# vinhisreal/YOLO-LitePi

Hardware: AMD Instinct MI355X
Metric: images/sec end-to-end (det+NMS+clf) 640x640 batch64 (higher is better)
Workload: dtype f16; 1 GPU; configs[2]: full det+NMS+ROI+ShuffleNetV2 pipeline, fp16, batch=64/GPU, 640x640, inputs resident in HBM; classifier=ShuffleNetV2 x1.0, 91 classes, seeded random weights, 64x64 ROIs, min_area=50, max_det=300, steps_in_flight=3, distinct_input_batches=4, global_batch=64, boxes_pre_area_filter_rank0=413

## Files before the change

yolo-litepi_amd/csrc/classifier.cpp:

```cpp
#include "classifier.h"

#include <algorithm>
#include <cmath>
#include <cstdlib>

namespace lp {

static const int kStageRepeats[3] = {4, 8, 4};
static const int kStageOut[3] = {116, 232, 464};

Classifier::Classifier(int prec, int impl, int max_rois, int num_classes, int input_size)
    : prec_(prec), impl_(impl), maxR_(max_rois), ncls_(num_classes), S_(input_size) {}

static View make_view(const DevBuf& buf, size_t es, int coff, int C, int pitch, int H, int W) {
  View v;
  v.base = static_cast<char*>(buf.p) + (size_t)coff * es;
  v.C = C; v.pitch = pitch; v.H = H; v.W = W;
  return v;
}

View Classifier::act_view(const Act& a, int coff, int C) const {
  return make_view(a.mem, prec_ == LP_FP16 ? 2 : 4, coff, C < 0 ? a.C : C, a.C, a.H, a.W);
}

// ... 143 lines not shown
        if (use_fused_) { upload_f32(fused_s2_[s].dw1, w); upload_f32(fused_s2_[s].dw1b, b); }
        Folded q = fold(sd, p + "branch1.2", p + "branch1.3");
        LP_CHECK(q.co == bf && q.ci == inp && q.k == 1, LP_ERR_ARG, "%sbranch1.2 shape", p.c_str());
        expand_pw(q, lin, 0, bfp, w, b, lin.Cp(), 0);
        B.b1_pw = add_pw(p + "branch1.2", w, b, lin.Cp(), bfp, ACT_RELU, Ho);
        if (use_fused_) { upload_u16(fused_s2_[s].pwb1, pack_fused_pw(w, bfp, lin.Cp())); upload_f32(fused_s2_[s].pwb1b, b); }
        Folded a1 = fold(sd, p + "branch2.0", p + "branch2.1");
        LP_CHECK(a1.co == bf && a1.ci == inp, LP_ERR_ARG, "%sbranch2.0 shape", p.c_str());
        expand_pw(a1, lin, 0, bfp, w, b, lin.Cp(), 0);
        B.b2_pw1 = add_pw(p + "branch2.0", w, b, lin.Cp(), bfp, ACT_RELU, Hin);
        if (use_fused_) { upload_u16(fused_s2_[s].pw1, pack_fused_pw(w, bfp, lin.Cp())); upload_f32(fused_s2_[s].pw1b, b); }
        b1dw_elems = std::max(b1dw_elems, (size_t)Ho * Ho * lin.Cp());
        b1_elems = std::max(b1_elems, (size_t)Ho * Ho * bfp);
        t1_elems = std::max(t1_elems, (size_t)Hin * Hin * bfp);
      } else {
        Folded a1 = fold(sd, p + "branch2.0", p + "branch2.1");
        LP_CHECK(a1.co == bf && a1.ci == bf, LP_ERR_ARG, "%sbranch2.0 shape", p.c_str());
        expand_pw(a1, lout, bf, bfp, w, b, bfp, bfp);
        B.b2_pw1 = add_pw(p + "branch2.0", w, b, bfp, bfp, ACT_RELU, Ho);
        t1_elems = std::max(t1_elems, (size_t)Ho * Ho * bfp);
        if (use_fused_) {
          fused_[s].emplace_back();
          upload_u16(fused_[s].back().w1, pack_fused_pw(w, bfp, bfp));
          upload_f32(fused_[s].back().b1, b);
        }
      }
      Layout lmid;
      lmid.C = bf;
      Folded d2 = fold(sd, p + "branch2.3", p + "branch2.4");
      LP_CHECK(d2.co == bf && d2.ci == 1 && d2.k == 3, LP_ERR_ARG, "%sbranch2.3 shape", p.c_str());
      expand_dw(d2, lmid, 0, bfp, 0, w, b);
      B.b2_dw = add_dw(p + "branch2.3", w, b, bfp, B.stride);
      if (use_fused_ && B.stride == 1) { upload_f32(fused_[s].back().dw, w); upload_f32(fused_[s].back().dwb, b); }
      if (use_fused_ && B.stride == 2) { upload_f32(fused_s2_[s].dw2, w); upload_f32(fused_s2_[s].dw2b, b); }
      Folded a2 = fold(sd, p + "branch2.5", p + "branch2.6");
      LP_CHECK(a2.co == bf && a2.ci == bf, LP_ERR_ARG, "%sbranch2.5 shape", p.c_str());
      expand_pw(a2, lmid, 0, bfp, w, b, bfp, 0);
      B.b2_pw2 = add_pw(p + "branch2.5", w, b, bfp, bfp, ACT_RELU, Ho);
      if (use_fused_ && B.stride == 1) { upload_u16(fused_[s].back().w2, pack_fused_pw(w, bfp, bfp)); upload_f32(fused_[s].back().b2, b); }
      if (use_fused_ && B.stride == 2) { upload_u16(fused_s2_[s].pw2, pack_fused_pw(w, bfp, bfp)); upload_f32(fused_s2_[s].pw2b, b); }
      t2_elems = std::max(t2_elems, (size_t)Ho * Ho * bfp);
      blocks_.push_back(B);
      inp = oup;
      lin = lout;
    }
    H = Ho;
    alloc_act(a_stage_[s][0], 2 * bfp, H, H);
    alloc_act(a_stage_[s][1], 2 * bfp, H, H);
  }
  if (use_fused_) {
    LP_CHECK(half_c_[0] == 58 && half_cp_[0] == 64 && half_c_[1] == 116 && half_cp_[1] == 128 && half_c_[2] == 232 && half_cp_[2] == 240,
             LP_ERR_STATE, "fused classifier kernels are built for ShuffleNetV2 x1.0 widths");
    a_x3_.alloc((size_t)maxR_ * 16 * 256 * 2);
  }
  const size_t es = prec_ == LP_FP16 ? 2 : 4;
  a_t1_.mem.alloc((size_t)maxR_ * t1_elems * es);
  a_t2_.mem.alloc((size_t)maxR_ * t2_elems * es);
  a_b1dw_.mem.alloc((size_t)maxR_ * b1dw_elems * es);
  a_b1_.mem.alloc((size_t)maxR_ * b1_elems * es);

  {
    Folded f = fold(sd, "conv5.0", "conv5.1");
    LP_CHECK(f.co == 1024 && f.ci == 464 && f.k == 1, LP_ERR_ARG, "conv5 must be 464->1024 1x1");
    std::vector<float> w, b;
    expand_pw(f, lin, 0, 1024, w, b, lin.Cp(), 0);
    conv5_ = add_pw("conv5.0", w, b, lin.Cp(), 1024, ACT_RELU, H);
    if (use_fused_) {
      LP_CHECK(H == 2, LP_ERR_STATE, "fused head expects a 2x2 stage-4 map");
      head_cin_p_ = lin.Cp();
      upload_u16(head_w5_, pack_fused_pw(w, 1024, lin.Cp()));
      upload_f32(head_b5_, b);
    }
    alloc_act(a_conv5_, 1024, H, H);
    alloc_act(a_mean_, 1024, 1, 1);
    const NamedTensor& fw = need(sd, "fc.weight");
    const NamedTensor& fb = need(sd, "fc.bias");
    LP_CHECK(fw.shape.size() == 2 && fw.shape[0] == ncls_ && fw.shape[1] == 1024 && (int)fb.numel() == ncls_, LP_ERR_ARG,
             "fc must be Linear(1024, %d), got [%lld,%lld]", ncls_, (long long)(fw.shape.size() ? fw.shape[0] : 0),
             (long long)(fw.shape.size() > 1 ? fw.shape[1] : 0));
    const int cp = round_up(ncls_, 8);
    lpitch_ = round_up(ncls_, 16);
    std::vector<float> w2((size_t)cp * 1024, 0.f), b2(cp, 0.f);
    for (int o = 0; o < ncls_; ++o) {
      memcpy(&w2[(size_t)o * 1024], fw.data + (size_t)o * 1024, 1024 * 4);
      b2[o] = fb.data[o];
    }
    fc_ = add_pw("fc", w2, b2, 1024, cp, ACT_NONE, 1);
    if (use_fused_) {
      head_nc_p_ = round_up(ncls_, 16);
      std::vector<float> wf((size_t)head_nc_p_ * 1024, 0.f), bf2(head_nc_p_, 0.f);
      for (int o = 0; o < ncls_; ++o) {
        memcpy(&wf[(size_t)o * 1024], fw.data + (size_t)o * 1024, 1024 * 4);
        bf2[o] = fb.data[o];
      }
      upload_u16(head_wfc_, pack_fused_pw(wf, head_nc_p_, 1024));
      upload_f32(head_bfc_, bf2);
    }
    d_logits_.alloc((size_t)maxR_ * lpitch_ * 4);
  }
  loaded_ = true;
}

void Classifier::forward(const uint8_t* rgb, const int* d_R, hipStream_t st, Profiler* prof, const Post* post) {
  LP_CHECK(loaded_, LP_ERR_STATE, "classifier not loaded");
  const size_t es = prec_ == LP_FP16 ? 2 : 4;
  const char* sfx = prec_ == LP_FP16 ? "_f16" : "_f32";
  const double esd = (double)es;
  auto P0 = [&]() { if (prof) prof->begin(st); };
  auto P1 = [&](const char* kname, const std::string& layer, double flops, double bytes) {
    if (prof) prof->end(st, std::string(kname) + sfx, layer, flops, bytes, true);
  };
  auto run_pw = [&](int idx, const View& in, const View& out, const View* x1, int half_c, int half_cp, int out_f32) {
    const ConvLayer& c = *pws_[idx];
    ConvIO io;
    io.in = in; io.out = out; io.N = maxR_; io.m_dyn = d_R; io.out_f32 = out_f32;
    if (x1) { io.x1 = *x1; io.half_c = half_c; io.half_cp = half_cp; }
    P0();
    c.launch(io, st);
    const double px = (double)out.H * out.W;
    P1(c.impl == IMPL_NAIVE ? "conv_naive" : "conv1x1_mfma", c.name, 2.0 * c.Cin * c.Cout * px,
       px * (c.Cin + c.Cout * (x1 ? 2.0 : 1.0)) * esd);
  };
  auto run_dw = [&](int idx, const View& in, const View& out) {
    const DwLayer& d = dws_[idx];
    P0();
    launch_dwconv3x3(prec_, in, out, d.w.as<float>(), d.b.as<float>(), d.stride, d_R, maxR_, st);
    P1("dwconv3x3", d.name, 2.0 * 9 * d.C * out.H * out.W, ((double)in.H * in.W + (double)out.H * out.W) * d.C * esd);
  };

  static const bool two_launch = getenv("LITEPI_CLS_LAYERWISE") == nullptr;
  if (use_fused_ && two_launch) {
    auto s2w = [](const FusedS2& f) {
      FusedS2W w;
      w.dw1 = f.dw1.as<float>(); w.dw1b = f.dw1b.as<float>(); w.pwb1 = f.pwb1.as<u32x4_t>(); w.pwb1b = f.pwb1b.as<float>();
      w.pw1 = f.pw1.as<u32x4_t>(); w.pw1b = f.pw1b.as<float>(); w.dw2 = f.dw2.as<float>(); w.dw2b = f.dw2b.as<float>();
      w.pw2 = f.pw2.as<u32x4_t>(); w.pw2b = f.pw2b.as<float>();
      return w;
    };
    auto s1w = [](const FusedW& f) {
      FusedBlockW w;
      w.w1 = f.w1.as<u32x4_t>(); w.b1 = f.b1.as<float>(); w.dw = f.dw.as<float>(); w.dwb = f.dwb.as<float>();
      w.w2 = f.w2.as<u32x4_t>(); w.b2 = f.b2.as<float>();
      return w;
    };
    ClsFrontArgs fa;
    memset(&fa, 0, sizeof(fa));
    fa.rgb = rgb; fa.m_dyn = d_R; fa.out = a_x3_.p;
    fa.stem_w = stem_frag_.as<u32x4_t>(); fa.stem_b = stem_bias4_.as<float>();
    fa.s20 = s2w(fused_s2_[0]);
    for (int q = 0; q < 3; ++q) fa.s2[q] = s1w(fused_[0][q]);
    fa.s30 = s2w(fused_s2_[1]);
    P0();
    launch_cls_front(fa, maxR_, st);
    P1("cls_front", "conv1..stage3.0", 2.0 * (0.66e6 + 2.10e6 + 0.60e6), 12288.0 + 8192.0);
    ClsBackArgs ba;
    memset(&ba, 0, sizeof(ba));
    ba.in = a_x3_.p; ba.m_dyn = d_R;
    for (int q = 0; q < 7; ++q) ba.s3[q] = s1w(fused_[1][q]);
    ba.s40 = s2w(fused_s2_[2]);
    for (int q = 0; q < 3; ++q) ba.s4[q] = s1w(fused_[2][q]);
    ba.w5 = head_w5_.as<u32x4_t>(); ba.b5 = head_b5_.as<float>();
    ba.wfc = head_wfc_.as<u32x4_t>(); ba.bfc = head_bfc_.as<float>();
    ba.nc = ncls_; ba.nc_p = head_nc_p_;
    ba.logits = d_logits_.as<float>(); ba.logits_pitch = lpitch_;
    if (post) {
      ba.probs = post->probs; ba.ids = post->ids; ba.dets = post->dets; ba.max_det = post->max_det;
      ba.roi_img = post->roi_img; ba.roi_slot = post->roi_slot;
    }
    P0();
    launch_cls_back(ba, maxR_, st);
    P1("cls_back", "stage3.1..softmax", 2.0 * (3.86e6 + 2.63e6 + 1.90e6 + 1024.0 * ncls_), 8192.0 + ncls_ * 4.0);
    return;
  }
  P0();
  launch_cls_stem(prec_, rgb, stem_w_.as<float>(), stem_b_.as<float>(), 24, act_view(a_stem_), S_, d_R, maxR_, st);
  P1("cls_stem", "conv1", 2.0 * 27 * 24 * a_stem_.H * a_stem_.W, (double)S_ * S_ * 3 + (double)a_stem_.H * a_stem_.W * 24 * esd);
  P0();
  launch_maxpool3x3s2(prec_, act_view(a_stem_), act_view(a_pool_), d_R, maxR_, st);
  P1("maxpool3x3s2", "maxpool", 0.0, ((double)a_stem_.H * a_stem_.W + (double)a_pool_.H * a_pool_.W) * 24 * esd);

  View x = act_view(a_pool_);
  size_t bi = 0;
  for (int s = 0; s < 3; ++s) {
    const int bf = half_c_[s], bfp = half_cp_[s];
    for (int r = 0; r < kStageRepeats[s]; ++r, ++bi) {
      const Block& B = blocks_[bi];
      if (use_fused_ && r == 1) {
        Act& dstf = a_stage_[s][1];
        FusedStageArgs fa;
        memset(&fa, 0, sizeof(fa));
        fa.in = x.base; fa.out = dstf.mem.p; fa.m_dyn = d_R;
        fa.nblk = kStageRepeats[s] - 1;
        for (int q = 0; q < fa.nblk; ++q) {
          const FusedW& fw = fused_[s][q];
          fa.blk[q].w1 = fw.w1.as<u32x4_t>(); fa.blk[q].b1 = fw.b1.as<float>();
          fa.blk[q].dw = fw.dw.as<float>(); fa.blk[q].dwb = fw.dwb.as<float>();
          fa.blk[q].w2 = fw.w2.as<u32x4_t>(); fa.blk[q].b2 = fw.b2.as<float>();
        }
        fa.HW = dstf.H * dstf.W; fa.W = dstf.W; fa.bf = bf; fa.bfp = bfp; fa.group = 64 / fa.HW;
        fa.in_pitch = x.pitch; fa.out_pitch = dstf.C;
        P0();
        launch_fused_stage(fa, maxR_, st);
        const double px = (double)fa.HW;
        P1("shuffle_stage_fused", fmt("stage%d.1-%d", s + 2, kStageRepeats[s] - 1),
           fa.nblk * (2.0 * 2.0 * bfp * bfp + 2.0 * 9 * bfp) * px, 2.0 * px * 2 * bfp * esd);
        x = act_view(dstf);
        bi += kStageRepeats[s] - 1;
        break;
      }
      Act& dst = a_stage_[s][r & 1];
      const int Ho = dst.H;
      const View out = act_view(dst);
      const View t2 = make_view(a_t2_.mem, es, 0, bfp, bfp, Ho, Ho);
      if (B.stride == 2) {
        const View b1dw = make_view(a_b1dw_.mem, es, 0, x.C, x.C, Ho, Ho);
        const View b1 = make_view(a_b1_.mem, es, 0, bfp, bfp, Ho, Ho);
        const View t1 = make_view(a_t1_.mem, es, 0, bfp, bfp, x.H, x.W);
        run_dw(B.b1_dw, x, b1dw);
        run_pw(B.b1_pw, b1dw, b1, nullptr, 0, 0, 0);
        run_pw(B.b2_pw1, x, t1, nullptr, 0, 0, 0);
        run_dw(B.b2_dw, t1, t2);
        run_pw(B.b2_pw2, t2, out, &b1, bf, bfp, 0);
      } else {
        const View x1 = View{x.base, bfp, x.pitch, x.H, x.W};
        const View x2 = View{static_cast<char*>(x.base) + (size_t)bfp * es, bfp, x.pitch, x.H, x.W};
        const View t1 = make_view(a_t1_.mem, es, 0, bfp, bfp, Ho, Ho);
        run_pw(B.b2_pw1, x2, t1, nullptr, 0, 0, 0);
        run_dw(B.b2_dw, t1, t2);
        run_pw(B.b2_pw2, t2, out, &x1, bf, bfp, 0);
      }
      x = out;
    }
  }
  if (use_fused_) {
    FusedHeadArgs ha;
    memset(&ha, 0, sizeof(ha));
    ha.in = x.base; ha.m_dyn = d_R; ha.in_pitch = x.pitch; ha.cin_p = head_cin_p_;
    ha.w5 = head_w5_.as<u32x4_t>(); ha.b5 = head_b5_.as<float>();
    ha.wfc = head_wfc_.as<u32x4_t>(); ha.bfc = head_bfc_.as<float>();
    ha.nc = ncls_; ha.nc_p = head_nc_p_;
    ha.logits = d_logits_.as<float>(); ha.logits_pitch = lpitch_;
    if (post) {
      ha.probs = post->probs; ha.ids = post->ids; ha.dets = post->dets; ha.max_det = post->max_det;
      ha.roi_img = post->roi_img; ha.roi_slot = post->roi_slot;
    }
    P0();
    launch_fused_head(ha, maxR_, st);
    P1("cls_head_fused", "conv5+mean+fc+softmax", 4.0 * 2.0 * head_cin_p_ * 1024 + 2.0 * 1024 * head_nc_p_,
       4.0 * head_cin_p_ * esd + ncls_ * 4.0);
    return;
  }
  run_pw(conv5_, x, act_view(a_conv5_), nullptr, 0, 0, 0);
  P0();
  launch_spatial_mean(prec_, act_view(a_conv5_), act_view(a_mean_), d_R, maxR_, st);
  P1("spatial_mean", "mean", 0.0, (double)(a_conv5_.H * a_conv5_.W + 1) * 1024 * esd);
  View lg;
  lg.base = d_logits_.p; lg.C = lpitch_; lg.pitch = lpitch_; lg.H = 1; lg.W = 1;
  run_pw(fc_, act_view(a_mean_), lg, nullptr, 0, 0, 1);
}

}
```

yolo-litepi_amd/csrc/cls_net.hip:

```cpp
#include "cls_net.h"

namespace lp {

typedef _Float16 half_t;
typedef _Float16 half8 __attribute__((ext_vector_type(8)));
typedef _Float16 half4 __attribute__((ext_vector_type(4)));
typedef _Float16 half2v __attribute__((ext_vector_type(2)));
typedef float floatx4 __attribute__((ext_vector_type(4)));
typedef uint32_t u32x4 __attribute__((ext_vector_type(4)));

#define CN_THREADS 512
#define CN_WAVES 8

#define BF2 58
#define BFP2 64
#define BF3 116
#define BFP3 128
#define BF4 232
#define BFP4 240

template <int SMAX>
__device__ __forceinline__ void wload(u32x4 (&af)[SMAX], const u32x4_t* __restrict__ w, int t, int S, int lane) {
#pragma unroll
  for (int s = 0; s < SMAX; ++s) {
// ... 42 lines not shown
}

template <int C, int WIN, int WOUT, int STRIDE>
__device__ __forceinline__ void dwconv(const char* in, int irow, char* out, int orow, const float* __restrict__ w,
                                       const float* __restrict__ b, int nroi, int tid) {
  constexpr int CG = C / 8;
  const int items = nroi * WOUT * WOUT * CG;
  for (int i = tid; i < items; i += CN_THREADS) {
    const int cg = i % CG, px = i / CG;
    const int r = px / (WOUT * WOUT), pp = px - r * (WOUT * WOUT);
    const int oy = pp / WOUT, ox = pp - oy * WOUT;
    float acc[8];
    {
      const floatx4 b0 = *reinterpret_cast<const floatx4*>(b + cg * 8), b1 = *reinterpret_cast<const floatx4*>(b + cg * 8 + 4);
#pragma unroll
      for (int j = 0; j < 4; ++j) { acc[j] = b0[j]; acc[4 + j] = b1[j]; }
    }
#pragma unroll 1
    for (int ky = 0; ky < 3; ++ky) {
      const int iy = oy * STRIDE - 1 + ky;
      if (iy < 0 || iy >= WIN) continue;
      const char* rowp = in + ((r * WIN + iy) * WIN) * irow + cg * 16;
      const float* wrow = w + (ky * 3) * C + cg * 8;
#pragma unroll
      for (int kx = 0; kx < 3; ++kx) {
        const int ix = ox * STRIDE - 1 + kx;
        const bool ok = ix >= 0 && ix < WIN;
        u32x4 raw = u32x4{0u, 0u, 0u, 0u};
        if (ok) raw = *reinterpret_cast<const u32x4*>(rowp + ix * irow);
        const half8 v = __builtin_bit_cast(half8, raw);
        const floatx4 w0 = *reinterpret_cast<const floatx4*>(wrow + kx * C);
        const floatx4 w1 = *reinterpret_cast<const floatx4*>(wrow + kx * C + 4);
#pragma unroll
        for (int j = 0; j < 4; ++j) {
          acc[j] = fmaf((float)v[j], w0[j], acc[j]);
          acc[4 + j] = fmaf((float)v[4 + j], w1[j], acc[4 + j]);
        }
      }
    }
    half8 o;
#pragma unroll
    for (int j = 0; j < 8; ++j) o[j] = (half_t)acc[j];
    *reinterpret_cast<half8*>(out + px * orow + cg * 16) = o;
  }
}

__device__ __forceinline__ int shuffle_phys(int l, int bf, int bfp) { return l < bf ? l : bfp + (l - bf); }

template <int BFP, int NB>
__device__ __forceinline__ void stage_biases(float* BI, const FusedBlockW* blk, int tid) {
  constexpr int Q = BFP / 4;
  for (int i = tid; i < NB * 2 * Q; i += CN_THREADS) {
    const int b = i / (2 * Q), rem = i - b * 2 * Q, which = rem / Q, j = rem - which * Q;
    const float* src = which ? blk[b].b2 : blk[b].b1;
    *reinterpret_cast<floatx4*>(BI + (size_t)(b * 2 + which) * BFP + 4 * j) = *reinterpret_cast<const floatx4*>(src + 4 * j);
  }
}

template <int C>
__device__ __forceinline__ void stage_dw(float* dst, const float* __restrict__ w, const float* __restrict__ b, int tid) {
  constexpr int Q = 10 * C / 4;
  for (int i = tid; i < Q; i += CN_THREADS)
    *reinterpret_cast<floatx4*>(dst + 4 * i) = i < 9 * C / 4 ? *reinterpret_cast<const floatx4*>(w + 4 * i) : *reinterpret_cast<const floatx4*>(b + 4 * (i - 9 * C / 4));
}

template <int BF, int BFP, int W, int PT, int ROUNDS, bool PREF = true>
__device__ __forceinline__ void s1_block(char* X, int xrow, char* T1, char* T2, int trow, const FusedBlockW& bw, const u32x4_t* w1n, int nroi,
                                         int p0, int tile0, int tstride, u32x4 (&f1)[ROUNDS][BFP / 32 + ((BFP % 32) ? 1 : 0)], int tid, float* DW, const float* BI) {
  constexpr int TT = BFP / 16, S = BFP / 32 + ((BFP % 32) ? 1 : 0);
  const int lane = tid & 63;
  const int g = lane >> 4, col = lane & 15;
  constexpr int NDW4 = 10 * BFP / 4, DWPT = (NDW4 + CN_THREADS - 1) / CN_THREADS;
  floatx4 dwreg[DWPT];
#pragma unroll
  for (int k = 0; k < DWPT; ++k) {
    int idx = tid + k * CN_THREADS;
    idx = idx < NDW4 ? idx : NDW4 - 1;
    dwreg[k] = idx < 9 * BFP / 4 ? *reinterpret_cast<const floatx4*>(bw.dw + 4 * idx) : *reinterpret_cast<const floatx4*>(bw.dwb + 4 * (idx - 9 * BFP / 4));
  }
  u32x4 f2[ROUNDS][S];
  floatx4 acc[ROUNDS][PT];
  int tc[ROUNDS];
  bool live[ROUNDS];
#pragma unroll
  for (int r = 0; r < ROUNDS; ++r) {
    const int t = tile0 + r * tstride;
    live[r] = t < TT;
    tc[r] = live[r] ? t : TT - 1;
  }
  if (PREF) {
#pragma unroll
    for (int r = 0; r < ROUNDS; ++r) wload<S>(f2[r], bw.w2, tc[r], S, lane);
  } else {
#pragma unroll
    for (int r = 0; r < ROUNDS; ++r) wload<S>(f1[r], bw.w1, tc[r], S, lane);
  }
#pragma unroll
  for (int r = 0; r < ROUNDS; ++r) {
    zero_acc<PT>(acc[r]);
    gemm_acc<S, PT>(f1[r], S, 0, X + BFP * 2, xrow, BFP, p0, lane, acc[r]);
    if (live[r]) store_relu<PT>(T1, trow, p0, tc[r], BI, acc[r], lane);
  }
  asm volatile("" ::: "memory");
  if (PREF) {
    if (w1n) {
#pragma unroll
      for (int r = 0; r < ROUNDS; ++r) wload<S>(f1[r], w1n, tc[r], S, lane);
    }
  } else {
#pragma unroll
    for (int r = 0; r < ROUNDS; ++r) wload<S>(f2[r], bw.w2, tc[r], S, lane);
  }
#pragma unroll
  for (int k = 0; k < DWPT; ++k) {
    const int idx = tid + k * CN_THREADS;
    if (idx < NDW4) *reinterpret_cast<floatx4*>(DW + 4 * idx) = dwreg[k];
  }
  __syncthreads();
  dwconv<BFP, W, W, 1>(T1, trow, T2, trow, DW, DW + 9 * BFP, nroi, tid);
  __syncthreads();
  half4 x1v[ROUNDS][PT];
#pragma unroll
  for (int r = 0; r < ROUNDS; ++r) {
    zero_acc<PT>(acc[r]);
    gemm_acc<S, PT>(f2[r], S, 0, T2, trow, BFP, p0, lane, acc[r]);
#pragma unroll
    for (int p = 0; p < PT; ++p) x1v[r][p] = *reinterpret_cast<const half4*>(X + (p0 + p * 16 + col) * xrow + (tc[r] * 16 + 4 * g) * 2);
  }
  __syncthreads();
#pragma unroll
  for (int r = 0; r < ROUNDS; ++r) {
    if (live[r]) {
      const int ch0 = tc[r] * 16 + 4 * g;
      const floatx4 bias = *reinterpret_cast<const floatx4*>(BI + BFP + ch0);
#pragma unroll
      for (int p = 0; p < PT; ++p) {
#pragma unroll
        for (int i = 0; i < 4; ++i) {
          const int c = ch0 + i;
          if (c < BF) {
            half2v pr;
            pr[0] = x1v[r][p][i];
            pr[1] = (half_t)fmaxf(acc[r][p][i] + bias[i], 0.f);
            *reinterpret_cast<half2v*>(X + (p0 + p * 16 + col) * xrow + shuffle_phys(2 * c, BF, BFP) * 2) = pr;
          }
        }
      }
    }
  }
  __syncthreads();
}

#define CF_IN 16
#define CF_RA 12352
#define CF_POOL (CF_RA + 49152)
#define CF_X2 (CF_POOL + 16384)
#define CF_LDS (CF_X2 + 17408)
#define CF_DW (10 * 64 * 4)
#define CF_BI (3 * 2 * 64 * 4)
#define CF_S2 ((10 * 24 + 10 * 64 + 10 * 128 + 10 * 128) * 4)
#define CF_POOLROW 64
#define CF_T1ROW 144
#define CF_X2ROW 272
#define CF_X3ROW 528

__global__ __launch_bounds__(CN_THREADS) void cls_front_kernel(const ClsFrontArgs a) {
  extern __shared__ __attribute__((aligned(16))) char smem[];
  const int tid0 = threadIdx.x, lane0 = tid0 & 63;
  const int R = *a.m_dyn;
  if ((int)blockIdx.x >= R) return;
  char* IN = smem + CF_IN;
  char* RA = smem + CF_RA;
  char* POOL = smem + CF_POOL;
  char* X2 = smem + CF_X2;
  char* T2 = smem;
  for (int i = tid0; i < 64 * CF_X2ROW / 16; i += CN_THREADS) *reinterpret_cast<u32x4*>(X2 + i * 16) = u32x4{0u, 0u, 0u, 0u};
  if (tid0 < 2) *reinterpret_cast<u32x4*>(smem + (tid0 ? CF_IN + 12288 : 0)) = u32x4{0u, 0u, 0u, 0u};
  stage_biases<BFP2, 3>(reinterpret_cast<float*>(smem + CF_LDS + CF_DW), a.s2, tid0);
  float* S2P = reinterpret_cast<float*>(smem + CF_LDS + CF_DW + CF_BI);
  stage_dw<24>(S2P, a.s20.dw1, a.s20.dw1b, tid0);
  stage_dw<64>(S2P + 240, a.s20.dw2, a.s20.dw2b, tid0);
  stage_dw<128>(S2P + 240 + 640, a.s30.dw1, a.s30.dw1b, tid0);
  stage_dw<128>(S2P + 240 + 640 + 1280, a.s30.dw2, a.s30.dw2b, tid0);
  const half8 sa0 = __builtin_bit_cast(half8, a.stem_w[lane0]), sa1 = __builtin_bit_cast(half8, a.stem_w[64 + lane0]);

  for (int r = blockIdx.x; r < R; r += gridDim.x) {
    int tid = tid0, lane = lane0;
    asm volatile("" : "+v"(tid), "+v"(lane));
    const int wave = __builtin_amdgcn_readfirstlane(tid >> 6);
    const int g = lane >> 4, col = lane & 15;
    {
      const u32x4* src = reinterpret_cast<const u32x4*>(a.rgb + (size_t)r * 12288);
      for (int i = tid; i < 768; i += CN_THREADS) *reinterpret_cast<u32x4*>(IN + i * 16) = src[i];
    }
    u32x4 fpw1[1];
    wload<1>(fpw1, a.s20.pw1, wave & 3, 1, lane);
    __syncthreads();

    for (int pt = wave * 8; pt < wave * 8 + 8; ++pt) {
      const int oy = pt >> 1, ox = (pt & 1) * 16 + col;
      const int b0 = 6 * ox - 3;
      uint32_t w0 = 0u, w1 = 0u;
      if (g < 3) {
        const int iy = 2 * oy - 1 + g;
        const int sh = b0 & 3, al = b0 - sh;
        const char* rowp = IN + (iy < 0 ? 0 : iy) * 192 + al;
        const uint32_t d0 = *reinterpret_cast<const uint32_t*>(rowp), d1 = *reinterpret_cast<const uint32_t*>(rowp + 4),
                       d2 = *reinterpret_cast<const uint32_t*>(rowp + 8);
        w0 = __builtin_amdgcn_alignbyte(d1, d0, sh);
        w1 = __builtin_amdgcn_alignbyte(d2, d1, sh);
        if (ox == 0) w0 &= 0xFF000000u;
        if (iy < 0) { w0 = 0u; w1 = 0u; }
      } else {
#pragma unroll
        for (int ky = 0; ky < 3; ++ky) {
          const int iy = 2 * oy - 1 + ky;
          const uint32_t v = iy < 0 ? 0u : (uint32_t) * reinterpret_cast<const uint8_t*>(IN + iy * 192 + b0 + 8);
          w0 |= v << (8 * ky);
        }
      }
      typedef uint32_t u32x4l __attribute__((ext_vector_type(4)));
      u32x4l hb;
      hb[0] = __builtin_amdgcn_perm(0x64646464u, w0, 0x04010400u);
      hb[1] = __builtin_amdgcn_perm(0x64646464u, w0, 0x04030402u);
      hb[2] = __builtin_amdgcn_perm(0x64646464u, w1, 0x04010400u);
      hb[3] = __builtin_amdgcn_perm(0x64646464u, w1, 0x04030402u);
      half8 bf = __builtin_bit_cast(half8, hb);
#pragma unroll
      for (int j = 0; j < 8; ++j) bf[j] = bf[j] - (half_t)1024.f;
      floatx4 c0 = floatx4{0.f, 0.f, 0.f, 0.f}, c1 = floatx4{0.f, 0.f, 0.f, 0.f};
      c0 = __builtin_amdgcn_mfma_f32_16x16x32_f16(sa0, bf, c0, 0, 0, 0);
      c1 = __builtin_amdgcn_mfma_f32_16x16x32_f16(sa1, bf, c1, 0, 0, 0);
      const int ci = (oy == 0 ? 1 : 0) | (ox == 0 ? 2 : 0);
      const floatx4 bb0 = *reinterpret_cast<const floatx4*>(a.stem_b + ci * 32 + 4 * g);
      char* o = RA + (oy * 32 + ox) * 48;
      half4 q;
#pragma unroll
      for (int i = 0; i < 4; ++i) q[i] = (half_t)fmaxf(c0[i] + bb0[i], 0.f);
      *reinterpret_cast<half4*>(o + 8 * g) = q;
      if (g < 2) {
        const floatx4 bb1 = *reinterpret_cast<const floatx4*>(a.stem_b + ci * 32 + 16 + 4 * g);
#pragma unroll
        for (int i = 0; i < 4; ++i) q[i] = (half_t)fmaxf(c1[i] + bb1[i], 0.f);
        *reinterpret_cast<half4*>(o + 32 + 8 * g) = q;
      }
    }
    __syncthreads();
    for (int i = tid; i < 768; i += CN_THREADS) {
      const int cg = i % 3, px = i / 3;
      const int oy = px >> 4, ox = px & 15;
      half8 m;
#pragma unroll
      for (int j = 0; j < 8; ++j) m[j] = (half_t)-65504.f;
#pragma unroll
      for (int ky = 0; ky < 3; ++ky) {
#pragma unroll
        for (int kx = 0; kx < 3; ++kx) {
          const int iy = 2 * oy - 1 + ky, ix = 2 * ox - 1 + kx;
          if (iy >= 0 && ix >= 0) {
            const half8 v = *reinterpret_cast<const half8*>(RA + (iy * 32 + ix) * 48 + cg * 16);
#pragma unroll
            for (int j = 0; j < 8; ++j) m[j] = v[j] > m[j] ? v[j] : m[j];
          }
        }
      }
      *reinterpret_cast<half8*>(POOL + px * CF_POOLROW + cg * 16) = m;
    }
    __syncthreads();

    char* T1 = RA;
    char* D1 = RA + 256 * CF_T1ROW;
    u32x4 fy[2];
    {
      const int t = wave & 3, p0 = (wave >> 2) * 128;
      floatx4 acc[8];
      zero_acc<8>(acc);
      gemm_acc<1, 8>(fpw1, 1, 0, POOL, CF_POOLROW, 24, p0, lane, acc);
      store_relu<8>(T1, CF_T1ROW, p0, t, a.s20.pw1b, acc, lane);
      if (wave < 4) wload<2>(fy, a.s20.pwb1, t, 1, lane); else wload<2>(fy, a.s20.pw2, t, 2, lane);
      dwconv<24, 16, 8, 2>(POOL, CF_POOLROW, D1, 64, S2P, S2P + 9 * 24, 1, tid);
    }
    __syncthreads();
    dwconv<64, 16, 8, 2>(T1, CF_T1ROW, T2, CF_T1ROW, S2P + 240, S2P + 240 + 9 * 64, 1, tid);
    __syncthreads();
    u32x4 f1[1][2];
    {
      const int t = wave & 3, which = wave >> 2;
      floatx4 acc[4];
      zero_acc<4>(acc);
      if (which == 0) gemm_acc<2, 4>(fy, 1, 0, D1, 64, 24, 0, lane, acc);
      else gemm_acc<2, 4>(fy, 2, 0, T2, CF_T1ROW, 64, 0, lane, acc);
      wload<2>(f1[0], a.s2[0].w1, t, 2, lane);
      const float* bias = which == 0 ? a.s20.pwb1b : a.s20.pw2b;
      const int ch0 = t * 16 + 4 * g;
      const floatx4 b = *reinterpret_cast<const floatx4*>(bias + ch0);
#pragma unroll
      for (int p = 0; p < 4; ++p) {
#pragma unroll
        for (int i = 0; i < 4; ++i) {
          const int c = ch0 + i;
          if (c < BF2)
            *reinterpret_cast<half_t*>(X2 + (p * 16 + col) * CF_X2ROW + shuffle_phys(2 * c + which, BF2, BFP2) * 2) =
                (half_t)fmaxf(acc[p][i] + b[i], 0.f);
        }
      }
    }
    __syncthreads();
#pragma unroll 1
    for (int b = 0; b < 3; ++b)
      s1_block<BF2, BFP2, 8, 2, 1>(X2, CF_X2ROW, RA, T2, CF_T1ROW, a.s2[b], b + 1 < 3 ? a.s2[b + 1].w1 : nullptr, 1, (wave >> 2) * 32, wave & 3,
                                   4, f1, tid, reinterpret_cast<float*>(smem + CF_LDS), reinterpret_cast<const float*>(smem + CF_LDS + CF_DW) + b * 2 * BFP2);

    char* T1c = RA;
    char* D1c = RA + 64 * CF_X2ROW;
    char* T2c = D1c + 16 * CF_X2ROW;
    char* X3 = T2c + 16 * CF_X2ROW;
    {
      u32x4 fa[4], fb[4], fc[4];
      wload<4>(fa, a.s30.pw1, wave, 4, lane);
      wload<4>(fb, a.s30.pwb1, wave, 4, lane);
      wload<4>(fc, a.s30.pw2, wave, 4, lane);
      for (int i = tid; i < 16 * CF_X3ROW / 16; i += CN_THREADS) *reinterpret_cast<u32x4*>(X3 + i * 16) = u32x4{0u, 0u, 0u, 0u};
      floatx4 acc[4];
      zero_acc<4>(acc);
      gemm_acc<4, 4>(fa, 4, 0, X2, CF_X2ROW, 128, 0, lane, acc);
      store_relu<4>(T1c, CF_X2ROW, 0, wave, a.s30.pw1b, acc, lane);
      dwconv<128, 8, 4, 2>(X2, CF_X2ROW, D1c, CF_X2ROW, S2P + 880, S2P + 880 + 9 * 128, 1, tid);
      __syncthreads();
      dwconv<128, 8, 4, 2>(T1c, CF_X2ROW, T2c, CF_X2ROW, S2P + 2160, S2P + 2160 + 9 * 128, 1, tid);
      __syncthreads();
      floatx4 y1[1], y2[1];
      zero_acc<1>(y1);
      zero_acc<1>(y2);
      gemm_acc<4, 1>(fb, 4, 0, D1c, CF_X2ROW, 128, 0, lane, y1);
      gemm_acc<4, 1>(fc, 4, 0, T2c, CF_X2ROW, 128, 0, lane, y2);
      const int ch0 = wave * 16 + 4 * g;
      const floatx4 b1 = *reinterpret_cast<const floatx4*>(a.s30.pwb1b + ch0), b2 = *reinterpret_cast<const floatx4*>(a.s30.pw2b + ch0);
#pragma unroll
      for (int i = 0; i < 4; ++i) {
        const int c = ch0 + i;
        if (c < BF3) {
          half2v pr;
          pr[0] = (half_t)fmaxf(y1[0][i] + b1[i], 0.f);
          pr[1] = (half_t)fmaxf(y2[0][i] + b2[i], 0.f);
          *reinterpret_cast<half2v*>(X3 + col * CF_X3ROW + shuffle_phys(2 * c, BF3, BFP3) * 2) = pr;
        }
      }
    }
    __syncthreads();
    {
      const int px = tid >> 5, ck = tid & 31;
      *reinterpret_cast<u32x4*>(reinterpret_cast<char*>(a.out) + ((size_t)r * 16 + px) * 512 + ck * 16) =
          *reinterpret_cast<const u32x4*>(X3 + px * CF_X3ROW + ck * 16);
    }
    __syncthreads();
  }
}

#define CB_RB 33792
#define CB_RC (CB_RB + 31744)
#define CB_X4 (CB_RC + 17408)
#define CB_LDS (CB_X4 + 15616)
#define CB_DW (10 * 240 * 4)
#define CB_BI3 (7 * 2 * 128 * 4)
#define CB_BI (CB_BI3 + 3 * 2 * 240 * 4)
#define CB_S2 ((10 * 256 + 10 * 240) * 4)
#define CB_T3ROW 272
#define CB_T4ROW 496
#define CB_X4ROW 976
#define CB_MROW 2064

__global__ __launch_bounds__(CN_THREADS) void cls_back_kernel(const ClsBackArgs a) {
  extern __shared__ __attribute__((aligned(16))) char smem[];
  const int tid0 = threadIdx.x, lane0 = tid0 & 63;
  const int R = *a.m_dyn;
  const int ngroups = (R + 3) >> 2;
  if ((int)blockIdx.x >= ngroups) return;
  char* X3 = smem;
  char* RB = smem + CB_RB;
  char* RC = smem + CB_RC;
  char* X4 = smem + CB_X4;
  for (int i = tid0; i < 16 * CB_X4ROW / 16; i += CN_THREADS) *reinterpret_cast<u32x4*>(X4 + i * 16) = u32x4{0u, 0u, 0u, 0u};
  stage_biases<BFP3, 7>(reinterpret_cast<float*>(smem + CB_LDS + CB_DW), a.s3, tid0);
  stage_biases<BFP4, 3>(reinterpret_cast<float*>(smem + CB_LDS + CB_DW + CB_BI3), a.s4, tid0);
  float* S2P = reinterpret_cast<float*>(smem + CB_LDS + CB_DW + CB_BI);
  stage_dw<256>(S2P, a.s40.dw1, a.s40.dw1b, tid0);
  stage_dw<240>(S2P + 2560, a.s40.dw2, a.s40.dw2b, tid0);

  for (int grp = blockIdx.x; grp < ngroups; grp += gridDim.x) {
    int tid = tid0, lane = lane0;
    asm volatile("" : "+v"(tid), "+v"(lane));
    const int wave = __builtin_amdgcn_readfirstlane(tid >> 6);
    const int g = lane >> 4, col = lane & 15;
    const int roi0 = grp * 4;
    const int nroi = (R - roi0) < 4 ? (R - roi0) : 4;
    u32x4 f3[1][4];
    wload<4>(f3[0], a.s3[0].w1, wave, 4, lane);
    for (int i = tid; i < 64 * 32; i += CN_THREADS) {
      const int px = i >> 5, ck = i & 31;
      u32x4 v = u32x4{0u, 0u, 0u, 0u};
      if (px < nroi * 16) v = *reinterpret_cast<const u32x4*>(reinterpret_cast<const char*>(a.in) + ((size_t)roi0 * 16 + px) * 512 + ck * 16);
      *reinterpret_cast<u32x4*>(X3 + px * CF_X3ROW + ck * 16) = v;
    }
    __syncthreads();
#pragma unroll 1
    for (int b = 0; b < 7; ++b)
      s1_block<BF3, BFP3, 4, 4, 1>(X3, CF_X3ROW, RB, RC, CB_T3ROW, a.s3[b], b + 1 < 7 ? a.s3[b + 1].w1 : nullptr, 4, 0, wave, 8, f3, tid,
                                   reinterpret_cast<float*>(smem + CB_LDS), reinterpret_cast<const float*>(smem + CB_LDS + CB_DW) + b * 2 * BFP3);

    char* T1 = RB;
    char* D1 = RC;
    char* T2 = RC + 16 * CF_X3ROW;
    u32x4 f4[2][8];
    {
      const int t0 = wave, t1 = wave + 8 < 15 ? wave + 8 : 14;
      const bool live1 = wave + 8 < 15;
      floatx4 y1[2][1];
      {
        u32x4 fb[2][8];
        wload<8>(fb[0], a.s40.pwb1, t0, 8, lane);
        wload<8>(fb[1], a.s40.pwb1, t1, 8, lane);
        dwconv<256, 4, 2, 2>(X3, CF_X3ROW, D1, CF_X3ROW, S2P, S2P + 9 * 256, 4, tid);
        __syncthreads();
        zero_acc<1>(y1[0]);
        zero_acc<1>(y1[1]);
        gemm_acc<8, 1>(fb[0], 8, 0, D1, CF_X3ROW, 256, 0, lane, y1[0]);
        gemm_acc<8, 1>(fb[1], 8, 0, D1, CF_X3ROW, 256, 0, lane, y1[1]);
      }
      asm volatile("" ::: "memory");
      {
        u32x4 fa[2][8];
        wload<8>(fa[0], a.s40.pw1, t0, 8, lane);
        wload<8>(fa[1], a.s40.pw1, t1, 8, lane);
        floatx4 acc[4];
        zero_acc<4>(acc);
        gemm_acc<8, 4>(fa[0], 8, 0, X3, CF_X3ROW, 256, 0, lane, acc);
        store_relu<4>(T1, CB_T4ROW, 0, t0, a.s40.pw1b, acc, lane);
        zero_acc<4>(acc);
        gemm_acc<8, 4>(fa[1], 8, 0, X3, CF_X3ROW, 256, 0, lane, acc);
        if (live1) store_relu<4>(T1, CB_T4ROW, 0, t1, a.s40.pw1b, acc, lane);
      }
      u32x4 fc[2][8];
      wload<8>(fc[0], a.s40.pw2, t0, 8, lane);
      wload<8>(fc[1], a.s40.pw2, t1, 8, lane);
      __syncthreads();
      dwconv<240, 4, 2, 2>(T1, CB_T4ROW, T2, CB_T4ROW, S2P + 2560, S2P + 2560 + 9 * 240, 4, tid);
      __syncthreads();
#pragma unroll
      for (int r = 0; r < 2; ++r) {
        const int t = r ? t1 : t0;
        floatx4 y2[1];
        zero_acc<1>(y2);
        gemm_acc<8, 1>(fc[r], 8, 0, T2, CB_T4ROW, 240, 0, lane, y2);
        if (r == 0 || live1) {
          const int ch0 = t * 16 + 4 * g;
          const floatx4 b1 = *reinterpret_cast<const floatx4*>(a.s40.pwb1b + ch0), b2 = *reinterpret_cast<const floatx4*>(a.s40.pw2b + ch0);
#pragma unroll
          for (int i = 0; i < 4; ++i) {
            const int c = ch0 + i;
            if (c < BF4) {
              half2v pr;
              pr[0] = (half_t)fmaxf(y1[r][0][i] + b1[i], 0.f);
              pr[1] = (half_t)fmaxf(y2[0][i] + b2[i], 0.f);
              *reinterpret_cast<half2v*>(X4 + col * CB_X4ROW + shuffle_phys(2 * c, BF4, BFP4) * 2) = pr;
            }
          }
        }
      }
      asm volatile("" ::: "memory");
      wload<8>(f4[0], a.s4[0].w1, t0, 8, lane);
      wload<8>(f4[1], a.s4[0].w1, t1, 8, lane);
    }
    __syncthreads();
#pragma unroll 1
    for (int b = 0; b < 3; ++b)
      s1_block<BF4, BFP4, 2, 1, 2, true>(X4, CB_X4ROW, RB, RB + 16 * CB_T4ROW, CB_T4ROW, a.s4[b], b + 1 < 3 ? a.s4[b + 1].w1 : nullptr, 4, 0, wave, 8, f4, tid,
                                         reinterpret_cast<float*>(smem + CB_LDS), reinterpret_cast<const float*>(smem + CB_LDS + CB_DW + CB_BI3) + b * 2 * BFP4);

    char* Mn = RC;
    float* LG = reinterpret_cast<float*>(RC + 4 * CB_MROW);
    {
      u32x4 fa[8], fb[8];
// ... 137 lines not shown
```

Baseline: 121,400 images/sec.

## Shrink cls_front LDS footprint to fit two workgroups per CU

Reorganizes the classifier front kernel's shared-memory map so regions alias (input/pool/T2 share one region, stem output and T1 share another) and the pool row pitch shrinks from 64 to 48 bytes. Stage-3 depthwise weights are no longer kept resident in LDS; each ROI prefetches them into registers and writes them into temporarily free scratch space. Static asserts keep total LDS under 80 KB so two 512-thread workgroups can co-reside per CU, with launch bounds raised to match. The cost is per-ROI re-zeroing and reloading of those weights, higher register pressure, and more fragile aliasing.

```diff
diff --git a/yolo-litepi_amd/csrc/classifier.cpp b/yolo-litepi_amd/csrc/classifier.cpp
--- a/yolo-litepi_amd/csrc/classifier.cpp
+++ b/yolo-litepi_amd/csrc/classifier.cpp
@@ -319,7 +319,7 @@
     fa.s30 = s2w(fused_s2_[1]);
     P0();
     launch_cls_front(fa, maxR_, st);
-    P1("cls_front", "conv1..stage3.0", 2.0 * (0.66e6 + 2.10e6 + 0.60e6), 12288.0 + 8192.0);
+    P1("cls_front", "conv1..stage3.0", 2.0 * (0.66e6 + 2.10e6 + 0.60e6), 12288.0 + 10240.0 + 8192.0);
     ClsBackArgs ba;
     memset(&ba, 0, sizeof(ba));
     ba.in = a_x3_.p; ba.m_dyn = d_R;
diff --git a/yolo-litepi_amd/csrc/cls_net.hip b/yolo-litepi_amd/csrc/cls_net.hip
--- a/yolo-litepi_amd/csrc/cls_net.hip
+++ b/yolo-litepi_amd/csrc/cls_net.hip
@@ -218,36 +218,42 @@
 }
 
 #define CF_IN 16
-#define CF_RA 12352
-#define CF_POOL (CF_RA + 49152)
-#define CF_X2 (CF_POOL + 16384)
+#define CF_R0SZ 14336
+#define CF_R1 CF_R0SZ
+#define CF_R1SZ 39936
+#define CF_X2 (CF_R1 + CF_R1SZ)
 #define CF_LDS (CF_X2 + 17408)
 #define CF_DW (10 * 64 * 4)
 #define CF_BI (3 * 2 * 64 * 4)
-#define CF_S2 ((10 * 24 + 10 * 64 + 10 * 128 + 10 * 128) * 4)
-#define CF_POOLROW 64
+#define CF_S2 ((10 * 24 + 10 * 64) * 4)
+#define CF_S3SET (10 * 128 * 4)
+#define CF_POOLROW 48
 #define CF_T1ROW 144
 #define CF_X2ROW 272
 #define CF_X3ROW 528
-
-__global__ __launch_bounds__(CN_THREADS) void cls_front_kernel(const ClsFrontArgs a) {
+#define CF_SA (64 * CF_T1ROW)
+#define CF_SB (CF_R1 + 96 * CF_X2ROW + 16 * CF_X3ROW)
+static_assert(CF_IN + 12288 + 16 <= CF_R0SZ && 256 * CF_POOLROW <= CF_R0SZ && CF_SA + CF_S3SET <= CF_R0SZ, "cls_front R0");
+static_assert(256 * CF_T1ROW + 64 * CF_POOLROW <= CF_R1SZ && CF_SB + CF_S3SET <= CF_R1 + CF_R1SZ, "cls_front R1");
+static_assert(32 * 32 * 48 <= CF_R1SZ + 17408, "STEM must fit R1 + R2");
+static_assert(CF_LDS + CF_DW + CF_BI + CF_S2 <= 81920, "cls_front: two workgroups per CU need <= 80 KB of LDS each");
+
+__global__ __launch_bounds__(CN_THREADS, 4) void cls_front_kernel(const ClsFrontArgs a) {
   extern __shared__ __attribute__((aligned(16))) char smem[];
   const int tid0 = threadIdx.x, lane0 = tid0 & 63;
   const int R = *a.m_dyn;
   if ((int)blockIdx.x >= R) return;
   char* IN = smem + CF_IN;
-  char* RA = smem + CF_RA;
-  char* POOL = smem + CF_POOL;
+  char* R1 = smem + CF_R1;
+  char* POOL = smem;
   char* X2 = smem + CF_X2;
   char* T2 = smem;
-  for (int i = tid0; i < 64 * CF_X2ROW / 16; i += CN_THREADS) *reinterpret_cast<u32x4*>(X2 + i * 16) = u32x4{0u, 0u, 0u, 0u};
-  if (tid0 < 2) *reinterpret_cast<u32x4*>(smem + (tid0 ? CF_IN + 12288 : 0)) = u32x4{0u, 0u, 0u, 0u};
   stage_biases<BFP2, 3>(reinterpret_cast<float*>(smem + CF_LDS + CF_DW), a.s2, tid0);
   float* S2P = reinterpret_cast<float*>(smem + CF_LDS + CF_DW + CF_BI);
   stage_dw<24>(S2P, a.s20.dw1, a.s20.dw1b, tid0);
   stage_dw<64>(S2P + 240, a.s20.dw2, a.s20.dw2b, tid0);
-  stage_dw<128>(S2P + 240 + 640, a.s30.dw1, a.s30.dw1b, tid0);
-  stage_dw<128>(S2P + 240 + 640 + 1280, a.s30.dw2, a.s30.dw2b, tid0);
+  const float* SA = reinterpret_cast<const float*>(smem + CF_SA);
+  const float* SB = reinterpret_cast<const float*>(smem + CF_SB);
   const half8 sa0 = __builtin_bit_cast(half8, a.stem_w[lane0]), sa1 = __builtin_bit_cast(half8, a.stem_w[64 + lane0]);
 
   for (int r = blockIdx.x; r < R; r += gridDim.x) {
@@ -256,6 +262,7 @@
     const int wave = __builtin_amdgcn_readfirstlane(tid >> 6);
     const int g = lane >> 4, col = lane & 15;
     {
+      if (tid < 2) *reinterpret_cast<u32x4*>(smem + (tid ? CF_IN + 12288 : 0)) = u32x4{0u, 0u, 0u, 0u};
       const u32x4* src = reinterpret_cast<const u32x4*>(a.rgb + (size_t)r * 12288);
       for (int i = tid; i < 768; i += CN_THREADS) *reinterpret_cast<u32x4*>(IN + i * 16) = src[i];
     }
@@ -299,7 +306,7 @@
       c1 = __builtin_amdgcn_mfma_f32_16x16x32_f16(sa1, bf, c1, 0, 0, 0);
       const int ci = (oy == 0 ? 1 : 0) | (ox == 0 ? 2 : 0);
       const floatx4 bb0 = *reinterpret_cast<const floatx4*>(a.stem_b + ci * 32 + 4 * g);
-      char* o = RA + (oy * 32 + ox) * 48;
+      char* o = R1 + (oy * 32 + ox) * 48;
       half4 q;
 #pragma unroll
       for (int i = 0; i < 4; ++i) q[i] = (half_t)fmaxf(c0[i] + bb0[i], 0.f);
@@ -324,7 +331,7 @@
         for (int kx = 0; kx < 3; ++kx) {
           const int iy = 2 * oy - 1 + ky, ix = 2 * ox - 1 + kx;
           if (iy >= 0 && ix >= 0) {
-            const half8 v = *reinterpret_cast<const half8*>(RA + (iy * 32 + ix) * 48 + cg * 16);
+            const half8 v = *reinterpret_cast<const half8*>(R1 + (iy * 32 + ix) * 48 + cg * 16);
 #pragma unroll
             for (int j = 0; j < 8; ++j) m[j] = v[j] > m[j] ? v[j] : m[j];
           }
@@ -334,8 +341,9 @@
     }
     __syncthreads();
 
-    char* T1 = RA;
-    char* D1 = RA + 256 * CF_T1ROW;
+    char* T1 = R1;
+    char* D1 = R1 + 256 * CF_T1ROW;
+    for (int i = tid; i < 64 * CF_X2ROW / 16; i += CN_THREADS) *reinterpret_cast<u32x4*>(X2 + i * 16) = u32x4{0u, 0u, 0u, 0u};
     u32x4 fy[2];
     {
       const int t = wave & 3, p0 = (wave >> 2) * 128;
@@ -344,17 +352,27 @@
       gemm_acc<1, 8>(fpw1, 1, 0, POOL, CF_POOLROW, 24, p0, lane, acc);
       store_relu<8>(T1, CF_T1ROW, p0, t, a.s20.pw1b, acc, lane);
       if (wave < 4) wload<2>(fy, a.s20.pwb1, t, 1, lane); else wload<2>(fy, a.s20.pw2, t, 2, lane);
-      dwconv<24, 16, 8, 2>(POOL, CF_POOLROW, D1, 64, S2P, S2P + 9 * 24, 1, tid);
+      dwconv<24, 16, 8, 2>(POOL, CF_POOLROW, D1, CF_POOLROW, S2P, S2P + 9 * 24, 1, tid);
     }
     __syncthreads();
     dwconv<64, 16, 8, 2>(T1, CF_T1ROW, T2, CF_T1ROW, S2P + 240, S2P + 240 + 9 * 64, 1, tid);
     __syncthreads();
     u32x4 f1[1][2];
+    floatx4 s3reg[2];
+#pragma unroll
+    for (int k = 0; k < 2; ++k) {
+      int i = tid + k * CN_THREADS;
+      i = i < 640 ? i : 639;
+      const int set = i >= 320, j = i - set * 320;
+      const float* w = set ? a.s30.dw2 : a.s30.dw1;
+      const float* bb = set ? a.s30.dw2b : a.s30.dw1b;
+      s3reg[k] = j < 288 ? *reinterpret_cast<const floatx4*>(w + 4 * j) : *reinterpret_cast<const floatx4*>(bb + 4 * (j - 288));
+    }
     {
       const int t = wave & 3, which = wave >> 2;
       floatx4 acc[4];
       zero_acc<4>(acc);
-      if (which == 0) gemm_acc<2, 4>(fy, 1, 0, D1, 64, 24, 0, lane, acc);
+      if (which == 0) gemm_acc<2, 4>(fy, 1, 0, D1, CF_POOLROW, 24, 0, lane, acc);
       else gemm_acc<2, 4>(fy, 2, 0, T2, CF_T1ROW, 64, 0, lane, acc);
       wload<2>(f1[0], a.s2[0].w1, t, 2, lane);
       const float* bias = which == 0 ? a.s20.pwb1b : a.s20.pw2b;
@@ -372,13 +390,18 @@
       }
     }
     __syncthreads();
+#pragma unroll
+    for (int k = 0; k < 2; ++k) {
+      const int i = tid + k * CN_THREADS;
+      if (i < 640) *reinterpret_cast<floatx4*>(smem + (i < 320 ? CF_SA + 16 * i : CF_SB + 16 * (i - 320))) = s3reg[k];
+    }
 #pragma unroll 1
     for (int b = 0; b < 3; ++b)
-      s1_block<BF2, BFP2, 8, 2, 1>(X2, CF_X2ROW, RA, T2, CF_T1ROW, a.s2[b], b + 1 < 3 ? a.s2[b + 1].w1 : nullptr, 1, (wave >> 2) * 32, wave & 3,
+      s1_block<BF2, BFP2, 8, 2, 1>(X2, CF_X2ROW, R1, T2, CF_T1ROW, a.s2[b], b + 1 < 3 ? a.s2[b + 1].w1 : nullptr, 1, (wave >> 2) * 32, wave & 3,
                                    4, f1, tid, reinterpret_cast<float*>(smem + CF_LDS), reinterpret_cast<const float*>(smem + CF_LDS + CF_DW) + b * 2 * BFP2);
 
-    char* T1c = RA;
-    char* D1c = RA + 64 * CF_X2ROW;
+    char* T1c = R1;
+    char* D1c = R1 + 64 * CF_X2ROW;
     char* T2c = D1c + 16 * CF_X2ROW;
     char* X3 = T2c + 16 * CF_X2ROW;
     {
@@ -391,9 +414,9 @@
       zero_acc<4>(acc);
       gemm_acc<4, 4>(fa, 4, 0, X2, CF_X2ROW, 128, 0, lane, acc);
       store_relu<4>(T1c, CF_X2ROW, 0, wave, a.s30.pw1b, acc, lane);
-      dwconv<128, 8, 4, 2>(X2, CF_X2ROW, D1c, CF_X2ROW, S2P + 880, S2P + 880 + 9 * 128, 1, tid);
+      dwconv<128, 8, 4, 2>(X2, CF_X2ROW, D1c, CF_X2ROW, SA, SA + 9 * 128, 1, tid);
       __syncthreads();
-      dwconv<128, 8, 4, 2>(T1c, CF_X2ROW, T2c, CF_X2ROW, S2P + 2160, S2P + 2160 + 9 * 128, 1, tid);
+      dwconv<128, 8, 4, 2>(T1c, CF_X2ROW, T2c, CF_X2ROW, SB, SB + 9 * 128, 1, tid);
       __syncthreads();
       floatx4 y1[1], y2[1];
       zero_acc<1>(y1);
```

Result: faster. 123,900 images/sec, median of 6 (+2.0%).
